# gallilmaimon/DISSC

Measured on AMD Instinct MI355X. Metric: audio-sec/sec (RTF) HiFi-GAN resynth, 10s x32 batch, higher is better.
Workload: dtype f32

## Files before the change

dissc_amd/csrc/respair.hip:

```cpp
#include "common.h"
#include "respair_f23.h"

namespace dissc {

template <int KS, int DIL, int NI>
__global__ void __launch_bounds__(256) respair16_kernel(const PairArgs a) {
  constexpr int C = 16, NW = 4, NT = 64 * NW;
  constexpr int SLOTS = 16 * NI * NW;
  constexpr int P2 = (KS - 1) / 2, P1 = P2 * DIL;
  constexpr int WOUT = (SLOTS - 2 * P2) & ~3;
  constexpr int XW1 = round32_16(3 + SLOTS + 2 * P1);
  constexpr int XW2 = round32_16(SLOTS + 2 * P2);
  constexpr int NV = XW1 / 4;
  constexpr int SV = (C * NV + NT - 1) / NT;
  constexpr int CW = 16 * NI + 4;
  constexpr int LPR = 4 * NI, RPP = 64 / LPR;
  static_assert(NW * 16 * CW <= C * XW1, "epilogue patches alias the input window");
  __shared__ __attribute__((aligned(16))) float Xs[C * XW1];
  __shared__ __attribute__((aligned(16))) float Ts[C * XW2];

  int b, len, o0;
  if (!pair_tile<WOUT>(a, gridDim.y, b, len, o0)) return;
  const int tid = threadIdx.x, lane = tid & 63, wave = tid >> 6;
  const int l15 = lane & 15, g = lane >> 4;
  const int tin0 = o0 - P2 - P1;
  const int tb = tin0 & ~3, sh = tin0 - tb;
  const float slope = a.slope;
  const float* xb = a.x + (size_t)b * a.bstride;

  f32x4 wa[KS];
  {
    const __amdgpu_buffer_rsrc_t w1r = wave_rsrc(a.w1, 0x7ffffff0u);
#pragma unroll
    for (int j = 0; j < KS; ++j) wa[j] = rsrc_load16(w1r, lane * 16u, j * 1024u);
  }
  const f32x4 bias1 = *reinterpret_cast<const f32x4*>(a.b1 + 4 * g);

  {
    f32x4 sv[SV];
    int r = tid / NV, v = tid - (tid / NV) * NV;
    constexpr int dr = NT / NV, dv = NT - dr * NV;
    int rr = r, vv = v;
#pragma unroll
    for (int i = 0; i < SV; ++i) {
      const int ci = rr < C ? rr : C - 1;
      int t = tb + 4 * vv;
      t = t < 0 ? 0 : (t > a.ld - 4 ? a.ld - 4 : t);
      sv[i] = *reinterpret_cast<const f32x4*>(xb + (size_t)ci * a.ld + t);
      vv += dv; rr += dr;
      if (vv >= NV) { vv -= NV; ++rr; }
    }
    rr = r; vv = v;
#pragma unroll
    for (int i = 0; i < SV; ++i) {
      if (rr < C) {
        const int t = tb + 4 * vv;
        f32x4 val = sv[i];
#pragma unroll
        for (int e = 0; e < 4; ++e) val[e] = ((t + e) >= 0 && (t + e) < len) ? lrelu(val[e], slope) : 0.f;
        *reinterpret_cast<f32x4*>(Xs + rr * XW1 + 4 * vv) = val;
      }
      vv += dv; rr += dr;
      if (vv >= NV) { vv -= NV; ++rr; }
    }
  }
  __syncthreads();

  f32x4 acc[NI];
#pragma unroll
  for (int ni = 0; ni < NI; ++ni) acc[ni] = f32x4{0.f, 0.f, 0.f, 0.f};
  {
    const float* bj = Xs + g * XW1 + sh + wave * (16 * NI) + l15;
#pragma unroll
    for (int j = 0; j < KS; ++j) {
#pragma unroll
      for (int cq = 0; cq < 4; ++cq)
#pragma unroll
        for (int ni = 0; ni < NI; ++ni)
          acc[ni] = __builtin_amdgcn_mfma_f32_16x16x4f32(wa[j][cq], bj[cq * 4 * XW1 + ni * 16 + j * DIL], acc[ni], 0, 0, 0);
      if (j & 1) __builtin_amdgcn_sched_barrier(0);
    }
  }
  f32x4 wb[KS];
  {
    const __amdgpu_buffer_rsrc_t w2r = wave_rsrc(a.w2, 0x7ffffff0u);
#pragma unroll
    for (int j = 0; j < KS; ++j) wb[j] = rsrc_load16(w2r, lane * 16u, j * 1024u);
  }
#pragma unroll
  for (int ni = 0; ni < NI; ++ni) {
    const int u = wave * (16 * NI) + ni * 16 + l15;
    const int t = o0 - P2 + u;
    const bool inside = t >= 0 && t < len;
#pragma unroll
    for (int r = 0; r < 4; ++r) {
      const float v = lrelu(acc[ni][r] + bias1[r], slope);
      Ts[(4 * g + r) * XW2 + u] = inside ? v : 0.f;
    }
  }
  __syncthreads();

#pragma unroll
  for (int ni = 0; ni < NI; ++ni) acc[ni] = f32x4{0.f, 0.f, 0.f, 0.f};
  const int prow = lane / LPR, pc4 = lane % LPR;
  const int ncol = wave * (16 * NI) + 4 * pc4;
  const int tcol = o0 + ncol;
  const size_t ob = (size_t)b * a.bstride;
  f32x4 rv[NI];
#pragma unroll
  for (int p = 0; p < NI; ++p) {
    const int row = p * RPP + prow;
    const int tc = tcol > a.ld - 4 ? a.ld - 4 : tcol;
    rv[p] = *reinterpret_cast<const f32x4*>(a.x + ob + (size_t)row * a.ld + tc);
  }
  {
    const float* bt = Ts + g * XW2 + wave * (16 * NI) + l15;
#pragma unroll
    for (int j = 0; j < KS; ++j) {
#pragma unroll
      for (int cq = 0; cq < 4; ++cq)
#pragma unroll
        for (int ni = 0; ni < NI; ++ni)
          acc[ni] = __builtin_amdgcn_mfma_f32_16x16x4f32(wb[j][cq], bt[cq * 4 * XW2 + ni * 16 + j], acc[ni], 0, 0, 0);
      if (j & 1) __builtin_amdgcn_sched_barrier(0);
    }
  }
  float* patch = Xs + wave * (16 * CW);
#pragma unroll
  for (int ni = 0; ni < NI; ++ni)
#pragma unroll
    for (int r = 0; r < 4; ++r) patch[(4 * g + r) * CW + ni * 16 + l15] = acc[ni][r];
  __builtin_amdgcn_wave_barrier();
  const int ehi = len - tcol < 4 ? len - tcol : 4;
  if (ncol < WOUT && tcol < len) {
#pragma unroll
    for (int p = 0; p < NI; ++p) {
      const int row = p * RPP + prow;
      f32x4 v = *reinterpret_cast<const f32x4*>(patch + row * CW + 4 * pc4);
      const size_t idx = ob + (size_t)row * a.ld + tcol;
      pair_store_tail(a, a.epi, idx, v, a.b2[row], rv[p], [&] { return load_quad(a.acc + idx); }, 0, ehi);
    }
  }
}

typedef float f32x16p __attribute__((ext_vector_type(16)));

template <int KS, int DIL, int NI>
__global__ void __launch_bounds__(256) respair32_kernel(const PairArgs a) {
  constexpr int C = 32, NW = 4, NT = 64 * NW;
  constexpr int SLOTS = 32 * NI * NW;
  constexpr int P2 = (KS - 1) / 2, P1 = P2 * DIL;
  constexpr int WOUT = (SLOTS - 2 * P2) & ~3;
  constexpr int XW1 = round32_16(3 + SLOTS + 2 * P1);
  constexpr int XW2 = round32_16(SLOTS + 2 * P2);
  constexpr int CW = 32 * NI + 4;
  constexpr int LPR = 8 * NI, RPP = 64 / LPR, NPASS = 8 / RPP;
  static_assert(XW2 <= XW1, "T fits the x window");
  __shared__ __attribute__((aligned(16))) float Xs[C * XW1];
  __shared__ __attribute__((aligned(16))) float Ps[NW * 8 * CW];
  float* const Ts = Xs;

  int b, len, o0;
  if (!pair_tile<WOUT>(a, gridDim.y, b, len, o0)) return;
  const int tid = threadIdx.x, lane = tid & 63, wave = tid >> 6;
  const int l31 = lane & 31, h = lane >> 5;
  const int tin0 = o0 - P2 - P1;
  const int tb = tin0 & ~3, sh = tin0 - tb;
  const float slope = a.slope;
  const float* xb = a.x + (size_t)b * a.bstride;
  const __amdgpu_buffer_rsrc_t w1p = wave_rsrc(a.w1, 0x7ffffff0u), w2p = wave_rsrc(a.w2, 0x7ffffff0u);
  const unsigned lane16 = lane * 16u;
  f32x4 av[2], avn[2];
  av[0] = rsrc_load16(w1p, lane16, 0);
  av[1] = rsrc_load16(w1p, lane16, 1024u);

  pair_stage_window<C, XW1, NT, 2>(a, xb, Xs, tb, len, tid);
  __syncthreads();

  f32x16p acc[NI];
#pragma unroll
  for (int ni = 0; ni < NI; ++ni)
#pragma unroll
    for (int e = 0; e < 16; ++e) acc[ni][e] = 0.f;

#define DISSC_PAIR32_TAPS(WP, BASE, XW, STEP, NEXT_WP)                                                     \
  _Pragma("unroll") for (int q = 0; q < 2 * KS; ++q) {                                                     \
    if (q + 1 < 2 * KS) {                                                                                  \
      avn[0] = rsrc_load16(WP, lane16, ((q + 1) * 2 + 0) * 1024u);                                         \
      avn[1] = rsrc_load16(WP, lane16, ((q + 1) * 2 + 1) * 1024u);                                         \
    } else {                                                                                               \
      avn[0] = rsrc_load16(NEXT_WP, lane16, 0);                                                            \
      avn[1] = rsrc_load16(NEXT_WP, lane16, 1024u);                                                        \
    }                                                                                                      \
    __builtin_amdgcn_sched_barrier(0);                                                                     \
    _Pragma("unroll") for (int hf = 0; hf < 2; ++hf)                                                       \
      _Pragma("unroll") for (int e = 0; e < 4; ++e)                                                        \
        _Pragma("unroll") for (int ni = 0; ni < NI; ++ni)                                                  \
          acc[ni] = __builtin_amdgcn_mfma_f32_32x32x2f32(                                                  \
              av[hf][e], BASE[((q / KS) * 16 + 2 * (4 * hf + e)) * XW + ni * 32 + (q % KS) * STEP], acc[ni], 0, 0, 0); \
    __builtin_amdgcn_sched_barrier(0);                                                                     \
    av[0] = avn[0];                                                                                        \
    av[1] = avn[1];                                                                                        \
  }

  {
    const float* bj = Xs + h * XW1 + sh + wave * (32 * NI) + l31;
    DISSC_PAIR32_TAPS(w1p, bj, XW1, DIL, w2p)
  }
  __syncthreads();
#pragma unroll
  for (int ni = 0; ni < NI; ++ni) {
    const int u = wave * (32 * NI) + ni * 32 + l31;
    const int t = o0 - P2 + u;
    const bool inside = t >= 0 && t < len;
#pragma unroll
    for (int r = 0; r < 16; ++r) {
      const int row = (r & 3) + 8 * (r >> 2) + 4 * h;
      const float v = lrelu(acc[ni][r] + a.b1[row], slope);
      Ts[row * XW2 + u] = inside ? v : 0.f;
    }
  }
  __syncthreads();
#pragma unroll
  for (int ni = 0; ni < NI; ++ni)
#pragma unroll
    for (int e = 0; e < 16; ++e) acc[ni][e] = 0.f;
  {
    const float* bt = Ts + h * XW2 + wave * (32 * NI) + l31;
    DISSC_PAIR32_TAPS(w2p, bt, XW2, 1, w2p)
  }
#undef DISSC_PAIR32_TAPS
  float* ep = Ps + wave * (8 * CW);
  const int prow = lane / LPR, pc4 = lane % LPR;
  const int ncol = wave * (32 * NI) + 4 * pc4;
  const int tcol = o0 + ncol;
  const size_t ob = (size_t)b * a.bstride;
  const bool live = ncol < WOUT && tcol < len;
  const int ehi = len - tcol < 4 ? len - tcol : 4;
#pragma unroll
  for (int qd = 0; qd < 4; ++qd) {
    f32x4 rv[NPASS];
#pragma unroll
    for (int p = 0; p < NPASS; ++p) {
      const int row = 8 * qd + p * RPP + prow;
      const int tc = tcol > a.ld - 4 ? a.ld - 4 : tcol;
      rv[p] = *reinterpret_cast<const f32x4*>(a.x + ob + (size_t)row * a.ld + tc);
    }
    __builtin_amdgcn_wave_barrier();
#pragma unroll
    for (int ni = 0; ni < NI; ++ni)
#pragma unroll
      for (int r = 0; r < 4; ++r) ep[(r + 4 * h) * CW + ni * 32 + l31] = acc[ni][4 * qd + r];
    __builtin_amdgcn_wave_barrier();
#pragma unroll
    for (int p = 0; p < NPASS; ++p) {
      const int prw = p * RPP + prow;
      f32x4 v = *reinterpret_cast<const f32x4*>(ep + prw * CW + 4 * pc4);
      if (!live) continue;
      const int row = 8 * qd + prw;
      const size_t idx = ob + (size_t)row * a.ld + tcol;
      pair_store_tail(a, a.epi, idx, v, a.b2[row], rv[p], [&] { return load_quad(a.acc + idx); }, 0, ehi);
    }
  }
}

template <int KS, int DIL>
static int launch_pair32(const PairArgs& a, int B, int Lmax, hipStream_t stream) {
  constexpr int NI = 2, SLOTS = 32 * NI * 4, WOUT = (SLOTS - (KS - 1)) & ~3;
  dim3 grid((Lmax + WOUT - 1) / WOUT, B);
  hipLaunchKernelGGL((respair32_kernel<KS, DIL, NI>), grid, dim3(256), 0, stream, a);
  DISSC_HIP_CHECK(hipGetLastError());
  return DISSC_OK;
}

template <int KS, int DIL>
static int launch_pair16(const PairArgs& a, int B, int Lmax, hipStream_t stream) {
  constexpr int NI = 4, SLOTS = 16 * NI * 4, WOUT = (SLOTS - (KS - 1)) & ~3;
  dim3 grid((Lmax + WOUT - 1) / WOUT, B);
  hipLaunchKernelGGL((respair16_kernel<KS, DIL, NI>), grid, dim3(256), 0, stream, a);
  DISSC_HIP_CHECK(hipGetLastError());
  return DISSC_OK;
}

bool respair_supported(int C, int KS, int dil) {
  if (C != 16 && C != 32) return false;
  return (KS == 3 || KS == 7 || KS == 11) && (dil == 1 || dil == 3 || dil == 5);
}

int launch_respair(const DevConv& c1, const DevConv& c2, const float* x, float* out, const Batch& bt, const EpiSpec& ep, int ld,
                   float slope, hipStream_t stream) {
  const int C = c1.M, B = bt.B, Lmax = bt.Lmax;
  if (!respair_supported(C, c1.KS, c1.dil) || c2.KS != c1.KS || c2.dil != 1 || c1.m32 != (C == 32) ||
      c2.m32 != (C == 32) || c1.prec || c2.prec || c1.CIN != C || c2.CIN != C || c2.M != C || ep.epi == EPI_STORE || x == out) {
    set_error("launch_respair: unsupported pair (C=%d k=%d d=%d)", C, c1.KS, c1.dil);
    return DISSC_EINVAL;
  }
  PairArgs a;
  a.x = x; a.out = out; a.acc = ep.acc; a.w1 = c1.wpack; a.w2 = c2.wpack; a.b1 = c1.bias; a.b2 = c2.bias;
  a.lengths = bt.lengths; a.len_default = bt.len_default; a.len_mul = bt.len_mul; a.ld = ld;
  a.bstride = (long long)C * ld; a.slope = slope; a.mrf_div = ep.mrf_div; a.epi = ep.epi; a.dbg = 0;
#define DISSC_PAIR16(K, D)                                                        \
  if (c1.KS == K && c1.dil == D)                                                  \
    return C == 16 ? launch_pair16<K, D>(a, B, Lmax, stream) : launch_pair32<K, D>(a, B, Lmax, stream);
  DISSC_PAIR16(3, 1) DISSC_PAIR16(3, 3) DISSC_PAIR16(3, 5)
  DISSC_PAIR16(7, 1) DISSC_PAIR16(7, 3) DISSC_PAIR16(7, 5)
  DISSC_PAIR16(11, 1) DISSC_PAIR16(11, 3) DISSC_PAIR16(11, 5)
#undef DISSC_PAIR16
  set_error("launch_respair: no instance");
  return DISSC_EINVAL;
}

}
```

dissc_amd/csrc/respair_f23.h:

```cpp
#pragma once
#include "common.h"
#include "ragged_epi.h"

namespace dissc {

struct PairArgs {
  const float* x;
  float* out;
  float* acc;
  const float* w1;
  const float* w2;
  const float* b1;
  const float* b2;
  const int32_t* lengths;
  int len_default, len_mul;
  int ld;
  long long bstride;
  float slope, mrf_div;
  int epi;
  int dbg;
};

template <int WOUT>
__device__ __forceinline__ bool pair_tile(const PairArgs& a, int B, int& b, int& len, int& o0) {
  if (a.lengths == nullptr) {
    b = blockIdx.y;
    len = a.len_default;
    o0 = blockIdx.x * WOUT;
    return o0 < len;
  }
  int tile;
  if (!ragged_tile<WOUT>(blockIdx.y * gridDim.x + blockIdx.x, B, [&](int i) { return a.lengths[i] * a.len_mul; }, b, tile, len))
    return false;
  o0 = tile * WOUT;
  return true;
}

template <int C, int XW, int NT, int NBATCH = 1>
__device__ __forceinline__ void pair_stage_window(const PairArgs& a, const float* xb, float* xs, int tb, int len, int tid) {
  constexpr int NV = XW / 4, NIT = ((C * NV + NT - 1) / NT + NBATCH - 1) / NBATCH;
  const float slope = a.slope;
#pragma unroll
  for (int nb = 0; nb < NBATCH; ++nb) {
    f32x4 sv[NIT];
#pragma unroll
    for (int it = 0; it < NIT; ++it) {
      const int i = tid + (nb * NIT + it) * NT;
      const int r = i / NV < C ? i / NV : C - 1, v = i - (i / NV) * NV;
      const int t = tb + 4 * v;
      const int tc = t < 0 ? 0 : (t > a.ld - 4 ? a.ld - 4 : t);
      sv[it] = *reinterpret_cast<const f32x4*>(xb + (size_t)r * a.ld + tc);
    }
#pragma unroll
    for (int it = 0; it < NIT; ++it) {
      const int i = tid + (nb * NIT + it) * NT;
      if (i >= C * NV) continue;
      const int r = i / NV, v = i - r * NV;
      const int t = tb + 4 * v;
      f32x4 val = sv[it];
#pragma unroll
      for (int e = 0; e < 4; ++e) val[e] = ((t + e) >= 0 && (t + e) < len) ? (val[e] > 0.f ? val[e] : val[e] * slope) : 0.f;
      *reinterpret_cast<f32x4*>(xs + r * XW + 4 * v) = val;
    }
  }
}

template <int C, int XW, int W1, int NT>
__device__ __forceinline__ void pair_zero_beyond_t(float* xs, int tid) {
  for (int i = tid; i < C * (XW - W1); i += NT) {
    const int r = i / (XW - W1), v = i - r * (XW - W1);
    xs[r * XW + W1 + v] = 0.f;
  }
}

template <class AccOld>
__device__ __forceinline__ void pair_store_tail(const PairArgs& a, int epi, size_t idx, f32x4 v, float bz, const f32x4& rv,
                                                AccOld acc_old, int elo, int ehi) {
  if (elo == 0 && ehi == 4) {
#pragma unroll
    for (int e = 0; e < 4; ++e) v[e] = (v[e] + bz) + rv[e];
    epi_store_res(epi, quad_at(a.out + idx), quad_at(a.acc + idx), v, acc_old, a.mrf_div);
  } else {
    for (int e = elo; e < ehi; ++e)
      epi_store_res(epi, a.out + idx + e, a.acc + idx + e, (v[e] + bz) + a.x[idx + e], [&] { return a.acc[idx + e]; }, a.mrf_div);
  }
}

template <int C_, int PROWS, int KS_, int DIL, int WCOLS = 64>
struct F23Geo {
  static constexpr int KS = KS_, NS = (KS_ + 2) / 3, C = C_, NW = 4;
  static constexpr int P2 = (KS - 1) / 2, P1 = P2 * DIL;
  static constexpr int D1 = DIL * NS, D2 = NS;
  static constexpr int NCOLS = WCOLS * NW;
  static constexpr int NU1 = NCOLS / D1, NC1 = NU1 * D1, W1 = 2 * NC1;
  static constexpr int NU2 = NCOLS / D2, NC2 = NU2 * D2, W2 = 2 * NC2;
  static constexpr int WOUT = ((W1 - 2 * P2) < W2 ? (W1 - 2 * P2) : W2) & ~3;
  static constexpr int REACH1 = (3 * NS - 1) * DIL, REACH2 = 3 * NS - 1;
  static constexpr int XW1 = round32_16(3 + W1 + REACH1);
  static constexpr int XW2 = round32_16(W2 + REACH2 + 1);
  static constexpr int XW = XW1 > XW2 ? XW1 : XW2;
  static constexpr int PW = 2 * WCOLS + 4;
  static_assert(NW * PROWS * PW <= C * XW, "the epilogue patches fit the buffer");
  static_assert(W1 <= XW && W2 + REACH2 < XW, "T fits the buffer");
};
template <int KS, int DIL> using F23Geo32 = F23Geo<32, 8, KS, DIL>;
template <int KS, int DIL> using F23Geo16 = F23Geo<16, 16, KS, DIL>;
template <int KS, int DIL> using F23Geo64 = F23Geo<64, 8, KS, DIL, 32>;

template <int C_, int KS_, int DIL_>
struct Tc6GeoC {
  static constexpr int KS = KS_, DIL = DIL_, NS = (KS_ + 3) / 4, C = C_, NW = 4, RB = C_ / 32, NCT = NW / RB;
  static constexpr int P2 = (KS - 1) / 2, P1 = P2 * DIL;
  static constexpr int D1 = DIL * NS, D2 = NS;
  static constexpr int NCOLS = 32 * NCT;
  static constexpr int NU1 = NCOLS / D1, NC1 = NU1 * D1, W1 = 3 * NC1;
  static constexpr int NCW2 = 32 / D2 * D2, OW = 3 * NCW2, W2 = NCT * OW;
  static constexpr int WOUT = ((W1 - 2 * P2) < W2 ? (W1 - 2 * P2) : W2) & ~3;
  static constexpr int REACH1 = (4 * NS - 1) * DIL, REACH2 = 4 * NS - 1;
  static constexpr int XW1 = (3 + W1 + REACH1 + 3) & ~3;
  static constexpr int XW2 = (W2 + REACH2 + 3) & ~3;
  static constexpr int XW = XW1 > XW2 ? XW1 : XW2;
  static constexpr int PW = 96 + 4;
  static constexpr int OCC = 3 * 4 * C * XW <= 160 * 1024 ? 3 : 2;
  static_assert(C == 32 || C == 64, "one or two 32-row blocks");
  static_assert(3 + OW <= PW - 1 && NW * 8 * PW <= C * XW, "the epilogue patches fit the buffer");
  static_assert(W1 <= XW && WOUT + 2 * P2 <= W1 && WOUT <= W2, "T fits the buffer and covers what the owned outputs read");
};
template <int KS, int DIL> using Tc6Geo = Tc6GeoC<32, KS, DIL>;
template <int KS, int DIL> using Tc6Geo64 = Tc6GeoC<64, KS, DIL>;

template <int KS, int DIL> __global__ void respair32_f23_kernel(const PairArgs a);
template <int KS, int DIL> __global__ void respair32_tc6_kernel(const PairArgs a);
template <int KS, int DIL> __global__ void respair16_f23_kernel(const PairArgs a);
template <int KS, int DIL> __global__ void respair64_f23_kernel(const PairArgs a);
template <int KS, int DIL> __global__ void respair64_tc6_kernel(const PairArgs a);
#if DISSC_EXPERIMENTAL
#define DISSC_PAIR_F23_SHAPES(X) X(11, 1) X(11, 3) X(11, 5) X(3, 1) X(3, 3) X(3, 5)
#else
#define DISSC_PAIR_F23_SHAPES(X) X(11, 1) X(11, 3) X(11, 5)
#endif
#define DISSC_PAIR_F23_C64_SHAPES(X) X(3, 1) X(3, 3) X(3, 5)
#define DISSC_PAIR_TC6_SHAPES(X) X(7, 1) X(7, 3) X(7, 5) X(11, 1) X(11, 3) X(11, 5)

}
```

Baseline: 10340.

## Reuse staged input quads as residual instead of reloading x in epilogue

The input-window staging now keeps in registers the raw quads that each thread's epilogue later needs as the residual. This removes the second global read of x in the fused residual-pair kernels. Staging is reorganised so owned quads are loaded per thread and only the halo is distributed across threads. It also adds a scheduling barrier on every tap for KS=11 and an early load of the accumulator for KS=7. The cost is higher register pressure from keeping the quads, and a stricter thread-to-quad mapping enforced by static asserts.

```diff
diff --git a/dissc_amd/csrc/respair.hip b/dissc_amd/csrc/respair.hip
--- a/dissc_amd/csrc/respair.hip
+++ b/dissc_amd/csrc/respair.hip
@@ -11,10 +11,10 @@
   constexpr int WOUT = (SLOTS - 2 * P2) & ~3;
   constexpr int XW1 = round32_16(3 + SLOTS + 2 * P1);
   constexpr int XW2 = round32_16(SLOTS + 2 * P2);
-  constexpr int NV = XW1 / 4;
-  constexpr int SV = (C * NV + NT - 1) / NT;
+  constexpr int Q0 = (P1 + P2 + 3) / 4;
   constexpr int CW = 16 * NI + 4;
   constexpr int LPR = 4 * NI, RPP = 64 / LPR;
+  static_assert(NI == C / 4 && LPR == 16 && RPP == 4, "the epilogue's quads are the ones pair_stage_window_keep keeps");
   static_assert(NW * 16 * CW <= C * XW1, "epilogue patches alias the input window");
   __shared__ __attribute__((aligned(16))) float Xs[C * XW1];
   __shared__ __attribute__((aligned(16))) float Ts[C * XW2];
@@ -36,34 +36,8 @@
   }
   const f32x4 bias1 = *reinterpret_cast<const f32x4*>(a.b1 + 4 * g);
 
-  {
-    f32x4 sv[SV];
-    int r = tid / NV, v = tid - (tid / NV) * NV;
-    constexpr int dr = NT / NV, dv = NT - dr * NV;
-    int rr = r, vv = v;
-#pragma unroll
-    for (int i = 0; i < SV; ++i) {
-      const int ci = rr < C ? rr : C - 1;
-      int t = tb + 4 * vv;
-      t = t < 0 ? 0 : (t > a.ld - 4 ? a.ld - 4 : t);
-      sv[i] = *reinterpret_cast<const f32x4*>(xb + (size_t)ci * a.ld + t);
-      vv += dv; rr += dr;
-      if (vv >= NV) { vv -= NV; ++rr; }
-    }
-    rr = r; vv = v;
-#pragma unroll
-    for (int i = 0; i < SV; ++i) {
-      if (rr < C) {
-        const int t = tb + 4 * vv;
-        f32x4 val = sv[i];
-#pragma unroll
-        for (int e = 0; e < 4; ++e) val[e] = ((t + e) >= 0 && (t + e) < len) ? lrelu(val[e], slope) : 0.f;
-        *reinterpret_cast<f32x4*>(Xs + rr * XW1 + 4 * vv) = val;
-      }
-      vv += dv; rr += dr;
-      if (vv >= NV) { vv -= NV; ++rr; }
-    }
-  }
+  f32x4 rv[NI];
+  pair_stage_window_keep<C, XW1, NT, Q0>(a, xb, Xs, tb, len, tid, rv);
   __syncthreads();
 
   f32x4 acc[NI];
@@ -78,7 +52,7 @@
 #pragma unroll
         for (int ni = 0; ni < NI; ++ni)
           acc[ni] = __builtin_amdgcn_mfma_f32_16x16x4f32(wa[j][cq], bj[cq * 4 * XW1 + ni * 16 + j * DIL], acc[ni], 0, 0, 0);
-      if (j & 1) __builtin_amdgcn_sched_barrier(0);
+      if ((j & 1) || KS == 11) __builtin_amdgcn_sched_barrier(0);
     }
   }
   f32x4 wb[KS];
@@ -106,12 +80,12 @@
   const int ncol = wave * (16 * NI) + 4 * pc4;
   const int tcol = o0 + ncol;
   const size_t ob = (size_t)b * a.bstride;
-  f32x4 rv[NI];
-#pragma unroll
-  for (int p = 0; p < NI; ++p) {
-    const int row = p * RPP + prow;
-    const int tc = tcol > a.ld - 4 ? a.ld - 4 : tcol;
-    rv[p] = *reinterpret_cast<const f32x4*>(a.x + ob + (size_t)row * a.ld + tc);
+  const bool live = ncol < WOUT && tcol < len;
+  constexpr bool ACC_EARLY = KS == 7;
+  f32x4 ao[NI];
+  if (ACC_EARLY && live && epi_rmw(a.epi)) {
+#pragma unroll
+    for (int p = 0; p < NI; ++p) ao[p] = load_quad(a.acc + ob + (size_t)(p * RPP + prow) * a.ld + tcol);
   }
   {
     const float* bt = Ts + g * XW2 + wave * (16 * NI) + l15;
@@ -132,13 +106,13 @@
     for (int r = 0; r < 4; ++r) patch[(4 * g + r) * CW + ni * 16 + l15] = acc[ni][r];
   __builtin_amdgcn_wave_barrier();
   const int ehi = len - tcol < 4 ? len - tcol : 4;
-  if (ncol < WOUT && tcol < len) {
+  if (live) {
 #pragma unroll
     for (int p = 0; p < NI; ++p) {
       const int row = p * RPP + prow;
       f32x4 v = *reinterpret_cast<const f32x4*>(patch + row * CW + 4 * pc4);
       const size_t idx = ob + (size_t)row * a.ld + tcol;
-      pair_store_tail(a, a.epi, idx, v, a.b2[row], rv[p], [&] { return load_quad(a.acc + idx); }, 0, ehi);
+      pair_store_tail<true>(a, a.epi, idx, v, a.b2[row], rv[p], [&] { return ACC_EARLY ? ao[p] : load_quad(a.acc + idx); }, 0, ehi);
     }
   }
 }
@@ -155,7 +129,9 @@
   constexpr int XW2 = round32_16(SLOTS + 2 * P2);
   constexpr int CW = 32 * NI + 4;
   constexpr int LPR = 8 * NI, RPP = 64 / LPR, NPASS = 8 / RPP;
+  constexpr int Q0 = (P1 + P2 + 3) / 4;
   static_assert(XW2 <= XW1, "T fits the x window");
+  static_assert(LPR == 16 && RPP == 4 && NPASS == 2, "the epilogue's quads are the ones pair_stage_window_keep keeps");
   __shared__ __attribute__((aligned(16))) float Xs[C * XW1];
   __shared__ __attribute__((aligned(16))) float Ps[NW * 8 * CW];
   float* const Ts = Xs;
@@ -174,7 +150,8 @@
   av[0] = rsrc_load16(w1p, lane16, 0);
   av[1] = rsrc_load16(w1p, lane16, 1024u);
 
-  pair_stage_window<C, XW1, NT, 2>(a, xb, Xs, tb, len, tid);
+  f32x4 xk[C / 4];
+  pair_stage_window_keep<C, XW1, NT, Q0>(a, xb, Xs, tb, len, tid, xk);
   __syncthreads();
 
   f32x16p acc[NI];
@@ -239,13 +216,6 @@
   const int ehi = len - tcol < 4 ? len - tcol : 4;
 #pragma unroll
   for (int qd = 0; qd < 4; ++qd) {
-    f32x4 rv[NPASS];
-#pragma unroll
-    for (int p = 0; p < NPASS; ++p) {
-      const int row = 8 * qd + p * RPP + prow;
-      const int tc = tcol > a.ld - 4 ? a.ld - 4 : tcol;
-      rv[p] = *reinterpret_cast<const f32x4*>(a.x + ob + (size_t)row * a.ld + tc);
-    }
     __builtin_amdgcn_wave_barrier();
 #pragma unroll
     for (int ni = 0; ni < NI; ++ni)
@@ -259,7 +229,7 @@
       if (!live) continue;
       const int row = 8 * qd + prw;
       const size_t idx = ob + (size_t)row * a.ld + tcol;
-      pair_store_tail(a, a.epi, idx, v, a.b2[row], rv[p], [&] { return load_quad(a.acc + idx); }, 0, ehi);
+      pair_store_tail<true>(a, a.epi, idx, v, a.b2[row], xk[NPASS * qd + p], [&] { return load_quad(a.acc + idx); }, 0, ehi);
     }
   }
 }
diff --git a/dissc_amd/csrc/respair_f23.h b/dissc_amd/csrc/respair_f23.h
--- a/dissc_amd/csrc/respair_f23.h
+++ b/dissc_amd/csrc/respair_f23.h
@@ -65,6 +65,46 @@
   }
 }
 
+template <int C, int XW, int NT, int Q0>
+__device__ __forceinline__ void pair_stage_window_keep(const PairArgs& a, const float* xb, float* xs, int tb, int len, int tid,
+                                                       f32x4 (&kept)[C / 4]) {
+  constexpr int NV = XW / 4, NH = NV - 64, NIT = (C * NH + NT - 1) / NT;
+  static_assert(NT == 256 && NH > 0 && Q0 >= 0 && Q0 <= NH, "four waves of 16 owned quads inside the window");
+  const float slope = a.slope;
+  const int lane = tid & 63, prow = lane >> 4;
+  const int vo = Q0 + (tid >> 6) * 16 + (lane & 15), to = tb + 4 * vo;
+  const int toc = to > a.ld - 4 ? a.ld - 4 : to;
+#pragma unroll
+  for (int j = 0; j < C / 4; ++j) kept[j] = *reinterpret_cast<const f32x4*>(xb + (size_t)(4 * j + prow) * a.ld + toc);
+  f32x4 sv[NIT];
+#pragma unroll
+  for (int it = 0; it < NIT; ++it) {
+    const int i = tid + it * NT;
+    const int r = i / NH < C ? i / NH : C - 1, hq = i - (i / NH) * NH;
+    const int t = tb + 4 * (hq < Q0 ? hq : hq + 64);
+    const int tc = t < 0 ? 0 : (t > a.ld - 4 ? a.ld - 4 : t);
+    sv[it] = *reinterpret_cast<const f32x4*>(xb + (size_t)r * a.ld + tc);
+  }
+#pragma unroll
+  for (int j = 0; j < C / 4; ++j) {
+    f32x4 val = kept[j];
+#pragma unroll
+    for (int e = 0; e < 4; ++e) val[e] = (to + e) < len ? (val[e] > 0.f ? val[e] : val[e] * slope) : 0.f;
+    *reinterpret_cast<f32x4*>(xs + (4 * j + prow) * XW + 4 * vo) = val;
+  }
+#pragma unroll
+  for (int it = 0; it < NIT; ++it) {
+    const int i = tid + it * NT;
+    if (i >= C * NH) continue;
+    const int r = i / NH, hq = i - r * NH;
+    const int v = hq < Q0 ? hq : hq + 64, t = tb + 4 * v;
+    f32x4 val = sv[it];
+#pragma unroll
+    for (int e = 0; e < 4; ++e) val[e] = ((t + e) >= 0 && (t + e) < len) ? (val[e] > 0.f ? val[e] : val[e] * slope) : 0.f;
+    *reinterpret_cast<f32x4*>(xs + r * XW + 4 * v) = val;
+  }
+}
+
 template <int C, int XW, int W1, int NT>
 __device__ __forceinline__ void pair_zero_beyond_t(float* xs, int tid) {
   for (int i = tid; i < C * (XW - W1); i += NT) {
@@ -73,7 +113,7 @@
   }
 }
 
-template <class AccOld>
+template <bool KEPT = false, class AccOld>
 __device__ __forceinline__ void pair_store_tail(const PairArgs& a, int epi, size_t idx, f32x4 v, float bz, const f32x4& rv,
                                                 AccOld acc_old, int elo, int ehi) {
   if (elo == 0 && ehi == 4) {
@@ -82,7 +122,8 @@
     epi_store_res(epi, quad_at(a.out + idx), quad_at(a.acc + idx), v, acc_old, a.mrf_div);
   } else {
     for (int e = elo; e < ehi; ++e)
-      epi_store_res(epi, a.out + idx + e, a.acc + idx + e, (v[e] + bz) + a.x[idx + e], [&] { return a.acc[idx + e]; }, a.mrf_div);
+      epi_store_res(epi, a.out + idx + e, a.acc + idx + e, (v[e] + bz) + (KEPT ? rv[e] : a.x[idx + e]),
+                    [&] { return a.acc[idx + e]; }, a.mrf_div);
   }
 }
 
```

Result: no change. 10390 (median of 6 runs) (+0.4%).
